# yang-song/score_sde_pytorch

Measured on AMD Instinct MI355X. Metric: pc_sampler_images_per_sec, higher is better.
Workload: dtype f32 via 3-way bf16 split, fp32 accumulate (the 1x1 / NIN / Linear GEMMs and the attention forward as exact-fp32 products on the BF16 matrix pipe, fp32 softmax; 3x3 convolutions and the attention backward on the fp32-MFMA kernels); 1 GPU; configs/ve/cifar10_ncsnpp_continuous PC sampler (reverse_diffusion+langevin), batch 256/GPU, N=1000, 32x32; 1 step = 1 PC iteration = 2 U-Net evaluations; batch_per_gpu=256, sde_steps=1000, state_finite=True, matrix_mode=bf16x6, parallelism=replicas x1 (no collectives)

## Files before the change

### score_sde_pytorch_amd/csrc/conv_mfma.hip

```cpp
#include "ssde_common.h"

typedef float f32x16 __attribute__((ext_vector_type(16)));

namespace {

struct ConvGeom {
  int N, Hin, Win, Hout, Wout, Cout, CoutPad;
  int stride, pad;
  int lTW, lTH;
  int tiles_x, tiles_per_img;
  int m_tiles, n_tiles;
};

struct ConvKParams {
  ssde_src main, aux;
  const float* w_main;
  const float* w_aux;
  ConvGeom g;
  const float* bias;
  const float* chan_add;
  int chan_add_ld;
  const float* resid;
  int resid_post;
  float scale;
  float* dst;
  float* gn_part;
  int ksplit;
  unsigned* sync;
};

constexpr int kThreads = 256;
#ifndef SSDE_CONV_BKC64
#define SSDE_CONV_BKC64 16
#endif

constexpr int kSyncSlots = 1 << 17;
__device__ unsigned g_conv_sync[kSyncSlots * 2];

template <int KS, int BKC, int BM, int BN, int TM, int TN, int MAXI>
__device__ __forceinline__ void conv_phase(const ssde_src& s, const float* __restrict__ wpk,
                                           const ConvGeom& g, int stride, int pad, int Hs, int Ws,
                                           int img0, int ty, int tx, int n0, int wm0, int wn0,
                                           f32x16 (&acc)[TM][TN], float* smem, int ks, int ksplit) {
  constexpr int T = KS * KS;
  constexpr int F4 = BKC / 4;
  constexpr int LDA = BKC + 4;
  constexpr int NB8 = BKC / 8;
  const int tid = threadIdx.x;
  const int lane = tid & 63;
  const int li = lane & 31, lh = lane >> 5;
  const int TW = 1 << g.lTW, TH = 1 << g.lTH;
// ... 258 lines not shown
#pragma unroll
      for (int it = 0; it < ITERS; ++it)
#pragma unroll
        for (int k = 0; k < 4; ++k)
          o[it][k] = dp[it] ? __hip_atomic_load(dp[it] + k, __ATOMIC_RELAXED, __HIP_MEMORY_SCOPE_AGENT) : 0.f;
#pragma unroll
      for (int it = 0; it < ITERS; ++it)
#pragma unroll
        for (int k = 0; k < 4; ++k) tp[it][k] += o[it][k];
    }
    if (first) {
      asm volatile("" ::: "memory");
      __builtin_amdgcn_s_waitcnt(0);
      __syncthreads();
      if (threadIdx.x == 0) atomicAdd(sy + 1, 1u);
      return;
    }
    __syncthreads();
    if (threadIdx.x == 0) { sy[0] = 0u; sy[1] = 0u; }
  }
  SsdeEpi e{p.bias, p.chan_add, p.chan_add_ld, p.resid, p.resid_post, p.scale, p.dst, g.Cout, p.gn_part};
  const int gn_entry = p.gn_part ? img0 * g.tiles_per_img + trem : -1;
  const int rpi_log2 = IMGS > 1 ? g.lTW + g.lTH : 30;
  ssde_store_tile<BM, BN, kThreads>(smem, LDT, n0, e, pixfn, gn_entry, rpi_log2, g.N * g.tiles_per_img);
}

struct TileCfg { int bm, bn; };
const TileCfg kTiles[5] = {{0, 0}, {256, 64}, {128, 64}, {64, 64}, {256, 32}};

struct ConvPlan {
  ConvKParams kp;
  int tile;
  int lds_bytes;
  int grid;
  bool has3, has1;
  int bkc;
  int gn_slices;
};

int src_check(const ssde_src& s, const char* what) {
  SSDE_REQUIRE(s.p0 != nullptr && s.c0 > 0, "conv: %s source missing", what);
  SSDE_REQUIRE(s.c0 % 4 == 0 && s.c1 % 4 == 0, "conv: %s channels must be multiples of 4 (got %d,%d)", what, s.c0, s.c1);
  SSDE_REQUIRE(s.c1 == 0 || s.p1 != nullptr, "conv: %s second tensor missing", what);
  SSDE_REQUIRE(s.c1 == 0 || s.c0 % 32 == 0, "conv: %s concat boundary must be a multiple of 32", what);
  if (s.pro_mode == SSDE_PRO_GN || s.pro_mode == SSDE_PRO_GN_SILU) {
    SSDE_REQUIRE(s.gn_groups > 0 && (s.c0 + s.c1) % s.gn_groups == 0 && ((s.c0 + s.c1) / s.gn_groups) % 4 == 0,
                 "conv: %s GroupNorm needs channels-per-group %% 4 == 0", what);
    SSDE_REQUIRE(s.gn_mean && s.gn_rstd && s.gn_gamma && s.gn_beta, "conv: %s GroupNorm pointers missing", what);
  }
  return SSDE_OK;
}

int pow2_floor(int v) { int p = 1; while (p * 2 <= v) p *= 2; return p; }

int halo_px(int bm, int w_out, int h_out, int stride, int ks, int* lTW, int* lTH) {
// ... 55 lines not shown
  } else {
    halo_px(kTiles[tile].bm, a->w_out, a->h_out, 1, 1, &lTW, &lTH);
  }
  const int bm = kTiles[tile].bm, bn = kTiles[tile].bn;
  const int tw = 1 << lTW, th = 1 << lTH, imgs = bm / (tw * th);

  ConvKParams& kp = pl->kp;
  kp.main = a->main; kp.aux = a->aux; kp.w_main = a->w_main; kp.w_aux = a->w_aux;
  ConvGeom& g = kp.g;
  g.N = a->n; g.Hin = a->h_in; g.Win = a->w_in; g.Hout = a->h_out; g.Wout = a->w_out;
  g.Cout = a->c_out; g.CoutPad = ssde_cdiv(a->c_out, 64) * 64;
  g.stride = pl->has3 ? a->stride : 1; g.pad = pl->has3 ? a->pad : 0;
  g.lTW = lTW; g.lTH = lTH;
  g.tiles_x = ssde_cdiv(a->w_out, tw);
  g.tiles_per_img = g.tiles_x * ssde_cdiv(a->h_out, th);
  g.m_tiles = ssde_cdiv(a->n, imgs) * g.tiles_per_img;
  g.n_tiles = ssde_cdiv(a->c_out, bn);
  kp.bias = a->bias; kp.chan_add = a->chan_add; kp.chan_add_ld = a->chan_add_ld;
  kp.resid = a->resid; kp.resid_post = a->resid_post; kp.scale = a->out_scale; kp.dst = a->dst;
  kp.gn_part = a->gn_part;
  const bool gn_ok = a->c_out % 4 == 0 && (imgs == 1 || (g.tiles_per_img == 1 && tw * th >= kThreads / (bn / 4)));
  pl->gn_slices = gn_ok ? g.tiles_per_img * (kThreads / 64) : 0;
  SSDE_REQUIRE(!a->gn_part || pl->gn_slices > 0, "conv: GroupNorm partials need one image per tile and c_out %% 4 == 0");

  int lds = 0;
  if (pl->has3) {
    const int px = imgs * ((th - 1) * g.stride + 3) * ((tw - 1) * g.stride + 3);
    const int lda = pl->bkc + 4;
    lds = (((px * lda + 3) & ~3) + 9 * bn * lda) * 4;
  }
  if (pl->has1) {
    const int l1 = (bm * 36 + bn * 36) * 4;
    if (l1 > lds) lds = l1;
  }
  const int epi_bytes = bm * (bn + 4) * 4 + 16;
  pl->lds_bytes = lds > epi_bytes ? lds : epi_bytes;
  pl->tile = tile;
  const bool split_ok = !(a->flags & SSDE_CONVF_NO_KSPLIT);
  const int wgs = ssde_cdiv(g.m_tiles, 8) * 8 * g.n_tiles;
  const int ctot = pl->has3 ? a->main.c0 + a->main.c1 : 0;
  kp.ksplit = (split_ok && pl->has3 && tile == SSDE_TILE_64x64 && wgs <= 320 && ctot >= 128 && a->c_out % 4 == 0 &&
               a->resid != a->dst && g.m_tiles * g.n_tiles <= kSyncSlots / 4) ? 2 : 1;
  kp.sync = nullptr;
  pl->grid = wgs * kp.ksplit;
  return SSDE_OK;
}

template <int WM, int WN, int TM, int TN, int BKC3 = 8>
int launch_cfg(ConvPlan& pl, hipStream_t st) {
  dim3 grid(pl.grid), block(kThreads);
  if (pl.kp.ksplit == 2) {
    pl.kp.sync = ssde_conv_sync_slots(pl.kp.g.m_tiles * pl.kp.g.n_tiles);
    SSDE_REQUIRE(pl.kp.sync, "conv: no hand-over slots for a split reduction");
  }
#define SSDE_CONV_LAUNCH(H3, H1)                                                                     \
  do {                                                                                               \
    auto kfn = conv_mfma_kernel<WM, WN, TM, TN, H3, H1, BKC3>;                                       \
    static std::atomic<bool> attr_set{false};             \
// ... 83 lines not shown
}

extern "C" int ssde_conv_gn_slices(const ssde_conv_args* a) {
  if (!a || a->c_out % 4 != 0) return 0;
  if (wino_pad_end_ok(a)) return 0;
  ssde_conv_args q = *a;
  q.gn_part = nullptr;
  if (ssde_wino_launcher fn = wino_launcher(q.tile)) {
    int s = 0;
    if (fn(&q, reinterpret_cast<void*>(1), &s)) return 0;
    return s;
  }
  if (q.dst && ssde_conv1x1_wants(&q)) {
    const int hw = q.h_out * q.w_out;
    if (hw % 64 == 0) return (hw / 64) * 4;
    return (hw >= 8 && hw < 64 && 64 % hw == 0) ? 4 : 0;
  }
  if (q.dst && ssde_conv_small_wants(&q)) return 0;
  ConvPlan pl;
  if (make_plan(&q, &pl)) return 0;
  return pl.gn_slices;
}

extern "C" int64_t ssde_conv_ws_floats(const ssde_conv_args* a) {
  if (int rc = wino_pad_end_ok(a)) return rc;
  if (a && a->tile == SSDE_TILE_WINOGRAD4P) return ssde_conv_wino4p_ws_floats(a);
  return 0;
}

extern "C" int ssde_conv_lds_bytes(const ssde_conv_args* a) {
  if (int rc = wino_pad_end_ok(a)) return rc;
  if (ssde_wino_launcher fn = a ? wino_launcher(a->tile) : nullptr) {
    int lds = 0;
    if (int rc = fn(a, nullptr, &lds)) return rc;
    return lds;
  }
  if (a && a->dst && ssde_conv1x1_wants(a)) {
    int lds = 0;
    if (int rc = ssde_conv1x1_launch(a, nullptr, &lds)) return rc;
    return lds;
  }
  if (a && a->dst && ssde_conv_small_wants(a)) {
    int lds = 0;
    if (int rc = ssde_conv_small_launch(a, nullptr, &lds)) return rc;
    return lds;
  }
// ... 5 lines not shown
```

### score_sde_pytorch_amd/csrc/conv_wino4p.hip

```cpp
#include "ssde_common.h"
#include <type_traits>

namespace {

typedef float f32x16 __attribute__((ext_vector_type(16)));

constexpr int kGemmWaves = 4;
constexpr int kBM = 64, kBN = 64;
constexpr int kKC = 4;
constexpr int kOutLdt = kBN + 4;

struct Wino4pGemmParams {
  const float* v;
  const float* u;
  float* m;
  int T, Q, Np, m_tiles, n_tiles, ks, qper;
};

__global__ __launch_bounds__(64 * kGemmWaves) void wino4p_gemm_kernel(const Wino4pGemmParams p) {
  const int lane = threadIdx.x & 63;
  int r = __builtin_amdgcn_readfirstlane((int)blockIdx.x * kGemmWaves + (int)(threadIdx.x >> 6));
  const int nt = r % p.n_tiles; r /= p.n_tiles;
  const int mt = r % p.m_tiles; r /= p.m_tiles;
  const int pos = r % 36, ks = r / 36;
// ... 101 lines not shown
#pragma unroll
  for (int px = 0; px < 6; ++px) {
    const float m0 = mm[px], m1 = mm[6 + px], m2 = mm[12 + px], m3 = mm[18 + px], m4 = mm[24 + px], m5 = mm[30 + px];
    const float s1 = m1 + m2, d1 = m1 - m2, s2 = m3 + m4, d2 = m3 - m4;
    const float tt[4] = {m0 + s1 + s2, d1 + 2.f * d2, s1 + 4.f * s2, d1 + 8.f * d2 + m5};
#pragma unroll
    for (int dy = 0; dy < 4; ++dy)
#pragma unroll
      for (int dx = 0; dx < 4; ++dx)
        if (kA[px][dx] != 0.f) y[dy][dx] += kA[px][dx] * tt[dy];
  }
#pragma unroll
  for (int dy = 0; dy < 4; ++dy)
#pragma unroll
    for (int dx = 0; dx < 4; ++dx) park[(dy * 4 + dx) * kOutLdt + lane] = y[dy][dx];
  SSDE_LDS_BARRIER();
  const int img = t / p.per_img, tr = t - img * p.per_img;
  const int ty = tr / p.tiles_w, tx = tr - ty * p.tiles_w;
  auto pixfn = [&](int row, size_t& pix, int& im) {
    im = img;
    pix = ((size_t)img * p.H + ty * 4 + (row >> 2)) * p.W + tx * 4 + (row & 3);
    return true;
  };
  ssde_store_tile<16, kBN, 64, 4, 0>(park, kOutLdt, n0, p.e, pixfn, p.e.gn_part ? t : -1);
}

struct W4pShape {
  int T, Q, Np, ks;
  int64_t v_floats;
  int64_t slab_floats;
};

bool w4p_legal_split(int Q, int ks) { return Q % (2 * kKC * ks) == 0; }

int w4p_splits(int waves1, int Q, unsigned flags) {
  if (flags & SSDE_CONVF_NO_KSPLIT) return 1;
  int ks = 1;
  if (flags & (SSDE_CONVF_KSPLIT2 | SSDE_CONVF_KSPLIT4)) {
    ks = (flags & SSDE_CONVF_KSPLIT4) ? 4 : 2;
  } else {
    const int simds = 4 * ssde_num_cus();
    ks = 4;
    while (ks > 1 && (waves1 * ks > simds || Q / ks < 8 * kKC)) ks /= 2;
  }
  while (ks > 1 && !w4p_legal_split(Q, ks)) ks /= 2;
  return ks;
}
// ... 17 lines not shown
  s->Np = ssde_cdiv(a->c_out, kBN) * kBN;
  s->ks = w4p_splits(36 * ssde_cdiv(s->T, kBM) * (s->Np / kBN), s->Q, a->flags);
  s->v_floats = (int64_t)36 * s->T * ctot;
  s->slab_floats = (int64_t)36 * s->T * s->Np;
  return SSDE_OK;
}

}

int64_t ssde_conv_wino4p_ws_floats(const ssde_conv_args* a) {
  W4pShape s;
  if (int rc = w4p_shape(a, &s)) return rc;
  return s.v_floats + s.ks * s.slab_floats;
}

int ssde_conv_wino4p_launch(const ssde_conv_args* a, void* stream, int* lds_out) {
  W4pShape s;
  if (int rc = w4p_shape(a, &s)) return rc;
  const int per_img = (a->h_out / 4) * (a->w_out / 4);
  if (lds_out && stream == reinterpret_cast<void*>(1)) {
    *lds_out = per_img;
    return SSDE_OK;
  }
  const int lds = 16 * kOutLdt * 4;
  if (lds_out) { *lds_out = lds; return SSDE_OK; }
  while (s.ks > 1 && a->wino_ws_floats < s.v_floats + s.ks * s.slab_floats) s.ks /= 2;
  SSDE_REQUIRE(a->wino_ws && a->wino_ws_floats >= s.v_floats + s.ks * s.slab_floats,
               "conv(winograd 4x4, position-batched): workspace (ssde_conv_args.wino_ws) missing or smaller than %lld floats",
               (long long)(s.v_floats + s.slab_floats));
  float* v = a->wino_ws;
  float* m = a->wino_ws + s.v_floats;
  ssde_conv_args x = *a;
  x.wino_v = v;
  if (int rc = ssde_wino4_xform_vq_launch(&x, stream)) return rc;
  hipStream_t st = static_cast<hipStream_t>(stream);
  const Wino4pGemmParams g{v, a->w_main, m, s.T, s.Q, s.Np, ssde_cdiv(s.T, kBM), s.Np / kBN, s.ks, s.Q / s.ks};
  const int waves = 36 * g.m_tiles * g.n_tiles * s.ks;
  hipLaunchKernelGGL(wino4p_gemm_kernel, dim3(ssde_cdiv(waves, kGemmWaves)), dim3(64 * kGemmWaves), 0, st, g);
  SSDE_LAUNCH_CHECK();
  Wino4pOutParams o;
  o.m = m; o.T = s.T; o.Np = s.Np; o.ks = s.ks;
  o.H = a->h_out; o.W = a->w_out; o.tiles_w = a->w_out / 4; o.per_img = per_img;
  o.e = SsdeEpi{a->bias, a->chan_add, a->chan_add_ld, a->resid, a->resid_post, a->out_scale, a->dst, a->c_out, a->gn_part};
  hipLaunchKernelGGL(wino4p_out_kernel, dim3(s.T, s.Np / kBN), dim3(64), lds, st, o);
  SSDE_LAUNCH_CHECK();
  return SSDE_OK;
}
```

### score_sde_pytorch_amd/csrc/conv_wino4r.hip

```cpp
#include "ssde_common.h"
#include <atomic>
#include <type_traits>

typedef float f32x16 __attribute__((ext_vector_type(16)));

#ifdef SSDE_W4R_TRACE
__device__ unsigned long long* g_w4r_trace;
extern "C" int ssde_debug_w4r_trace(void* buf) {
  return hipMemcpyToSymbol(HIP_SYMBOL(g_w4r_trace), &buf, sizeof(buf)) == hipSuccess ? 0 : -5;
}
#define SSDE_RT(slot)                                                                                     \
  do {                                                                                                    \
    if (tr_on) g_w4r_trace[tr_base + (slot)] = __builtin_amdgcn_s_memtime();                              \
  } while (0)
#else
#define SSDE_RT(slot) do { } while (0)
#endif

namespace {

constexpr int kNP = 9;
constexpr int kNV = 5;
constexpr int kPos = 36, kTiles = 32;
constexpr int kURegion = kNP * 32 * 4;
constexpr int kUFloats = 8 * kURegion;
constexpr int kWaves = 8, kThreads = 64 * kWaves, kBN = 64;
constexpr int kLdm = kBN + 2, kLdt = kBN + 4;
constexpr int kLds = kPos * 16 * kLdm * 4;
static_assert(256 * kLdt <= kPos * 16 * kLdm, "parked tile");

struct Wino4rParams {
  const float* v;
  const float* wpk;
  int N, H, W, Cout, Ctot;
  int lTWt, lTHt;
  int tiles_x, tiles_per_img, m_tiles, n_tiles;
  const float* bias; const float* chan_add; int chan_add_ld;
  const float* resid; int resid_post;
  float scale;
  float* dst;
  float* gn_part;
  int T, tiles_h, tiles_w;
  int ksplit;
  unsigned* sync;
  int ticket_off;
};

template <int kKs>
__global__ __launch_bounds__(kThreads, 2) void conv_wino4r_kernel(const Wino4rParams p) {
  constexpr bool kSplit = kKs > 1;
  SSDE_LDS(smem);
  const int tid = threadIdx.x, lane = tid & 63;
  const int wave = __builtin_amdgcn_readfirstlane(tid >> 6);
  const int li = lane & 31, lh = lane >> 5;
  auto pos_of = [&](int i) { return i < 4 ? 4 * wave + i : 32 + (wave >> 1); };
  const int TWt = 1 << p.lTWt, THt = 1 << p.lTHt;
  const int IMGS = kTiles >> (p.lTWt + p.lTHt);
  const size_t v_stage = (size_t)p.T * 16;
  const size_t u_stage = (size_t)p.n_tiles * kUFloats * 4;
  const uint32_t u_off = (uint32_t)lane * 16u, u_off8 = 2048u + (uint32_t)lane * 8u;
  ssde_f32x2 va[2][kNV], u2[2];
  ssde_f32x4 u4[2][4];
  uint32_t v_off[kNV];
  const char* vs = nullptr;
  const char* us = nullptr;
#define SSDE_W4R_ROUND_AT(S, VN, UN)                                                               \
  do {                                                                                             \
    SSDE_GLOAD8_I_SAFE(va[S][0], v_off[0], VN, 0); SSDE_GLOAD16_I_SAFE(u4[S][0], u_off, UN, -2048);          \
// ... 80 lines not shown
    SSDE_W4R_POS(S, 3, 1024);
    SSDE_WAIT_VMCNT_FOR(kMode == 0 ? 18 : kMode == 1 ? 10 : 0, va[S][4], u2[S]);
    SSDE_W4R_MFMA(S, 4, 8, u2[S].x, u2[S].y);
    __builtin_amdgcn_sched_barrier(0);
    if (kMode == 0) { SSDE_W4R_LOADV(S, 4); SSDE_GLOAD8_I(u2[S], u_off8, un, 0); }
    __builtin_amdgcn_sched_barrier(0);
  };
  {
    using S0 = std::integral_constant<int, 0>; using S1 = std::integral_constant<int, 1>;
    using Steady = std::integral_constant<int, 0>; using Penult = std::integral_constant<int, 1>; using Last = std::integral_constant<int, 2>;
    int st = 0;
    for (; st + 3 < nst; st += 2) { stage(S0{}, Steady{}, st); stage(S1{}, Steady{}, st + 1); }
    stage(S0{}, Penult{}, st);
    stage(S1{}, Last{}, st + 1);
  }
#undef SSDE_W4R_POS
#undef SSDE_W4R_MFMA
#undef SSDE_W4R_LOADV
  SSDE_RT(3);

  SsdeEpi e{p.bias, p.chan_add, p.chan_add_ld, p.resid, p.resid_post, p.scale, p.dst, p.Cout, p.gn_part};
  const int gn_base = !p.gn_part ? -1 : (IMGS == 1 ? (img0 * p.tiles_per_img + trem) * 2 : img0);
  const int rpi_log2 = IMGS > 2 ? 8 - (4 - p.lTWt - p.lTHt) : 30;
  const int li_e = tid & 31, lh_e = (tid >> 5) & 1;
  const int e_tl = tid / (kBN / 2), e_cp = tid % (kBN / 2);
  float* park = smem;
#pragma unroll
  for (int rnd = 0; rnd < 2; ++rnd) {
    auto pixfn = [&](int row, size_t& pix, int& img) {
      const int tile = rnd * 16 + (row >> 4), dy = (row >> 2) & 3, dx = row & 3;
      const int il = tile >> (p.lTWt + p.lTHt);
      const int tr = (tile >> p.lTWt) & (THt - 1), tc = tile & (TWt - 1);
      img = img0 + il;
      const int oy = (ty * THt + tr) * 4 + dy, ox = (tx * TWt + tc) * 4 + dx;
      if (img >= p.N || oy >= p.H || ox >= p.W) return false;
      pix = ((size_t)img * p.H + oy) * p.W + ox;
      return true;
    };
#pragma unroll
    for (int j = 0; j < kNP; ++j)
#pragma unroll
      for (int r8 = 0; r8 < 8; ++r8) {
        const int r = rnd * 8 + r8;
        const int tl = (r & 3) + 4 * lh_e + 8 * ((r >> 2) & 1);
        const int pos = pos_of(j >> 1), half = j < 8 ? (j & 1) : (wave & 1);
        smem[(pos * 16 + tl) * kLdm + half * 32 + li_e] = acc[j][r];
// ... 128 lines not shown
  SSDE_REQUIRE((s.c0 + s.c1) % 8 == 0, "conv(winograd 4x4, register-fed): input channels must be a multiple of 8 (the stage loop runs in pairs)");
  Wino4rParams p;
  p.v = a->wino_v; p.wpk = a->w_main;
  p.N = a->n; p.H = a->h_out; p.W = a->w_out; p.Cout = a->c_out; p.Ctot = s.c0 + s.c1;
  const int twt = pow2_floor((a->w_out / 4) < 8 ? (a->w_out / 4) : 8);
  int tht = kTiles / twt; if (tht > a->h_out / 4) tht = a->h_out / 4;
  tht = pow2_floor(tht);
  const int imgs = kTiles / (twt * tht);
  p.lTWt = ssde_ilog2(twt); p.lTHt = ssde_ilog2(tht);
  p.tiles_x = ssde_cdiv(a->w_out, 4 * twt);
  p.tiles_per_img = p.tiles_x * ssde_cdiv(a->h_out, 4 * tht);
  p.m_tiles = ssde_cdiv(a->n, imgs) * p.tiles_per_img;
  p.n_tiles = ssde_cdiv(a->c_out, kBN);
  p.bias = a->bias; p.chan_add = a->chan_add; p.chan_add_ld = a->chan_add_ld;
  p.resid = a->resid; p.resid_post = a->resid_post; p.scale = a->out_scale; p.dst = a->dst;
  p.gn_part = a->gn_part;
  p.tiles_h = a->h_out / 4; p.tiles_w = a->w_out / 4; p.T = a->n * p.tiles_h * p.tiles_w;
  const bool gn_ok = a->c_out % 4 == 0 && (imgs == 1 || (p.tiles_per_img == 1 && imgs <= 8));
  SSDE_REQUIRE(!a->gn_part || gn_ok, "conv(winograd 4x4, register-fed): GroupNorm partials not available for this tiling");
  if (lds_out && stream == reinterpret_cast<void*>(1)) {
    *lds_out = gn_ok ? (imgs == 1 ? 2 * p.tiles_per_img : 1) * (kThreads / 64) : 0;
    return SSDE_OK;
  }
  p.ticket_off = kLds / 4;
  const int lds = kLds + 16;
  SSDE_REQUIRE(lds <= 160 * 1024, "conv(winograd 4x4, register-fed): %d bytes of LDS", lds);
  if (lds_out) { *lds_out = lds; return SSDE_OK; }
  SSDE_REQUIRE(a->wino_v, "conv(winograd 4x4, register-fed): the transformed-input buffer (ssde_conv_args.wino_v) is missing");
  SSDE_REQUIRE(36ull * (unsigned long long)p.T * (unsigned)p.Ctot * 4ull < (1ull << 32),
               "conv(winograd 4x4, register-fed): a transformed input of 4 GB or more is not addressable by this kernel");
  const int wgs = ssde_cdiv(p.m_tiles, 8) * 8 * p.n_tiles;
  p.ksplit = a->resid != a->dst ? ssde_conv_wino4r_splits(wgs, p.Ctot, a->c_out, a->flags) : 1;
  p.sync = p.ksplit > 1 ? ssde_conv_sync_slots(p.m_tiles * p.n_tiles) : nullptr;
  if (!p.sync) p.ksplit = 1;
  const dim3 grid(wgs * p.ksplit);
  auto go = [&](auto kfn, std::atomic<bool>& attr_set) {
    if (!attr_set) {
      if (hipFuncSetAttribute(reinterpret_cast<const void*>(kfn), hipFuncAttributeMaxDynamicSharedMemorySize, 160 * 1024) != hipSuccess)
        return false;
      attr_set = true;
    }
    hipLaunchKernelGGL(kfn, grid, dim3(kThreads), lds, static_cast<hipStream_t>(stream), p);
    return true;
  };
  static std::atomic<bool> set[3];
  const bool ok = p.ksplit == 4 ? go(conv_wino4r_kernel<4>, set[2]) : p.ksplit == 2 ? go(conv_wino4r_kernel<2>, set[1])
// ... 6 lines not shown
```

### score_sde_pytorch_amd/csrc/runtime.hip

```cpp
#include "ssde_common.h"
#include <string.h>
#include <vector>

static thread_local char g_err[512] = "";

void ssde_set_error(const char* fmt, ...) {
  va_list ap;
  va_start(ap, fmt);
  vsnprintf(g_err, sizeof(g_err), fmt, ap);
  va_end(ap);
}

extern "C" const char* ssde_last_error(void) { return g_err; }

int ssde_num_cus() {
  if (const char* e = getenv("SSDE_NUM_CUS")) { const int v = atoi(e); if (v > 0) return v; }
  constexpr int kMaxDev = 64;
  static std::atomic<int> cus[kMaxDev];
  int dev = 0;
  if (hipGetDevice(&dev) != hipSuccess || dev < 0 || dev >= kMaxDev) dev = 0;
  int c = cus[dev].load(std::memory_order_relaxed);
  if (c <= 0) {
    int v = 0;
    if (hipDeviceGetAttribute(&v, hipDeviceAttributeMultiprocessorCount, dev) != hipSuccess || v <= 0) v = 256;
// ... 50 lines not shown
    case SSDE_OP_COLSUM: return ssde_colsum(&op.u.colsum, stream);
    case SSDE_OP_GN_BWD_REDUCE: return ssde_gn_bwd_reduce(&op.u.gn_bwd, stream);
    case SSDE_OP_PROLOGUE_BWD: return ssde_prologue_bwd(&op.u.pro_bwd, stream);
    case SSDE_OP_ATTN_BWD: return ssde_attention_bwd(&op.u.attn_bwd, stream);
    case SSDE_OP_PERTURB: return ssde_perturb(&op.u.perturb, stream);
    case SSDE_OP_DSM_LOSS: return ssde_dsm_loss(&op.u.dsm_loss, stream);
    case SSDE_OP_SUMSQ_FLAT: return ssde_sumsq_flat(&op.u.sumsq_flat, stream);
    case SSDE_OP_ADAM: return ssde_adam_clip_ema(&op.u.adam, stream);
    case SSDE_OP_MEMSET: return ssde_memset(&op.u.memset, stream);
    case SSDE_OP_AXPY: return ssde_axpy(&op.u.axpy, stream);
    case SSDE_OP_PACK: return ssde_pack_weights(&op.u.pack, stream);
    case SSDE_OP_GN_FINALIZE: return ssde_gn_finalize(&op.u.gn_fin, stream);
    case SSDE_OP_PF_DRIFT: return ssde_pf_drift(&op.u.pf_drift, stream);
    case SSDE_OP_HUTCH_DIV: return ssde_hutch_div(&op.u.hutch_div, stream);
    case SSDE_OP_COLSUM_FINISH: return ssde_colsum_finish(&op.u.colsum_fin, stream);
    case SSDE_OP_GN_BWD_FINISH: return ssde_gn_bwd_finish(&op.u.gn_bwd_fin, stream);
    case SSDE_OP_GN_APPLY: return ssde_gn_apply(&op.u.gn_apply, stream);
    case SSDE_OP_GN_APPLY_BWD: return ssde_gn_apply_bwd(&op.u.gn_apply_bwd, stream);
  }
  ssde_set_error("program: unknown op kind %d", op.kind);
  return SSDE_EINVAL;
}

extern "C" int ssde_program_run(const ssde_op* ops, int32_t n_ops, void* stream) {
  SSDE_REQUIRE(ops && n_ops >= 0, "program: null ops");
  for (int i = 0; i < n_ops; ++i) {
    if (int rc = run_one(ops[i], stream)) {
      char tmp[400];
      strncpy(tmp, g_err, sizeof(tmp) - 1); tmp[sizeof(tmp) - 1] = 0;
      ssde_set_error("op %d (kind %d): %s", i, ops[i].kind, tmp);
      return rc;
    }
  }
  return SSDE_OK;
}

extern "C" int ssde_program_run_timed(const ssde_op* ops, int32_t n_ops, void* stream, float* ms) {
  SSDE_REQUIRE(ops && n_ops >= 0 && ms, "program: null args");
  hipStream_t st = static_cast<hipStream_t>(stream);
  std::vector<hipEvent_t> ev(n_ops + 1);
  for (auto& e : ev) SSDE_HIP_CHECK(hipEventCreate(&e));
  int rc = SSDE_OK;
  SSDE_HIP_CHECK(hipEventRecord(ev[0], st));
  for (int i = 0; i < n_ops && rc == SSDE_OK; ++i) {
    rc = run_one(ops[i], stream);
    if (rc == SSDE_OK && hipEventRecord(ev[i + 1], st) != hipSuccess) { ssde_set_error("hipEventRecord failed"); rc = SSDE_EHIP; }
  }
  if (rc == SSDE_OK) {
    if (hipStreamSynchronize(st) != hipSuccess) { ssde_set_error("hipStreamSynchronize failed"); rc = SSDE_EHIP; }
    for (int i = 0; i < n_ops && rc == SSDE_OK; ++i)
      if (hipEventElapsedTime(&ms[i], ev[i], ev[i + 1]) != hipSuccess) { ssde_set_error("hipEventElapsedTime failed"); rc = SSDE_EHIP; }
  }
  for (auto& e : ev) hipEventDestroy(e);
  return rc;
}

struct SsdeGraph { hipGraph_t graph; hipGraphExec_t exec; };

extern "C" int ssde_graph_capture(const ssde_op* ops, int32_t n_ops, void* stream, void** graph_out) {
  SSDE_REQUIRE(ops && graph_out, "graph: null args");
  hipStream_t st = static_cast<hipStream_t>(stream);
  SSDE_REQUIRE(st != nullptr, "graph: capture needs a non-default stream");
  SSDE_HIP_CHECK(hipStreamBeginCapture(st, hipStreamCaptureModeThreadLocal));
  int rc = ssde_program_run(ops, n_ops, stream);
  hipGraph_t graph = nullptr;
  hipError_t e = hipStreamEndCapture(st, &graph);
  if (rc != SSDE_OK) { if (graph) hipGraphDestroy(graph); return rc; }
  if (e != hipSuccess) { ssde_set_error("hipStreamEndCapture failed: %s", hipGetErrorString(e)); return SSDE_EHIP; }
  hipGraphExec_t exec = nullptr;
// ... 23 lines not shown
```

### score_sde_pytorch_amd/csrc/ssde_common.h

```cpp
#pragma once
#include <hip/hip_runtime.h>
#include <stdint.h>
#include <stdio.h>
#include <stdarg.h>
#include <stdlib.h>
#include <atomic>
#include "../../include/ssde.h"

#define SSDE_OK 0
#define SSDE_EINVAL (-22)
#define SSDE_EHIP (-5)

void ssde_set_error(const char* fmt, ...);
int ssde_conv_wino_launch(const ssde_conv_args* a, void* stream, int* lds_out);
int ssde_conv_wino4_launch(const ssde_conv_args* a, void* stream, int* lds_out);
bool ssde_wino4_xform_merges_gn(const ssde_conv_args* a);
int ssde_wino4_xform_vq_launch(const ssde_conv_args* a, void* stream);
int ssde_conv_wino4r_launch(const ssde_conv_args* a, void* stream, int* lds_out);
int ssde_conv_wino4p_launch(const ssde_conv_args* a, void* stream, int* lds_out);
int64_t ssde_conv_wino4p_ws_floats(const ssde_conv_args* a);
bool ssde_conv1x1_wants(const ssde_conv_args* a);
int ssde_conv1x1_launch(const ssde_conv_args* a, void* stream, int* lds_out);
unsigned* ssde_conv_sync_slots(int need);
int ssde_conv_wino4_splits(int wgs, int ctot, int c_out, unsigned flags);
int ssde_conv_wino4r_splits(int wgs, int ctot, int c_out, unsigned flags);
bool ssde_conv_small_wants(const ssde_conv_args* a);
int ssde_conv_small_launch(const ssde_conv_args* a, void* stream, int* lds_out);
bool ssde_wgrad_wino_wants(const ssde_wgrad_args* a);
int64_t ssde_wgrad_wino_scratch_floats(const ssde_wgrad_args* a);
int ssde_wgrad_wino_launch(const ssde_wgrad_args* a, void* stream);
bool ssde_wgrad_wino4_wants(const ssde_wgrad_args* a);
int64_t ssde_wgrad_wino4_scratch_floats(const ssde_wgrad_args* a);
int ssde_wgrad_wino4_launch(const ssde_wgrad_args* a, void* stream);

#define SSDE_REQUIRE(cond, ...)            \
  do {                                     \
    if (!(cond)) {                         \
      ssde_set_error(__VA_ARGS__);         \
      return SSDE_EINVAL;                  \
    }                                      \
  } while (0)

#define SSDE_HIP_CHECK(expr)                                                        \
  do {                                                                              \
    hipError_t _e = (expr);                                                         \
// ... 129 lines not shown
__device__ __forceinline__ float ssde_keep(uint32_t elem, const SsdePro& p) {
  return ssde_hash32(elem * 0x9E3779B1u + p.key) >= p.thresh ? p.dscale : 0.f;
}
__device__ __forceinline__ float4 ssde_pro_apply(float4 v, float mu, float rs, const float4& gam, const float4& bet,
                                                 uint32_t elem0, const SsdePro& p) {
  if (p.gn) {
    v.x = (v.x - mu) * rs * gam.x + bet.x;
    v.y = (v.y - mu) * rs * gam.y + bet.y;
    v.z = (v.z - mu) * rs * gam.z + bet.z;
    v.w = (v.w - mu) * rs * gam.w + bet.w;
  }
  if (p.silu) { v.x = ssde_silu(v.x); v.y = ssde_silu(v.y); v.z = ssde_silu(v.z); v.w = ssde_silu(v.w); }
  if (__builtin_expect(p.drop, 0)) {
    v.x *= ssde_keep(elem0, p); v.y *= ssde_keep(elem0 + 1u, p);
    v.z *= ssde_keep(elem0 + 2u, p); v.w *= ssde_keep(elem0 + 3u, p);
  }
  return v;
}

struct SsdeEpi {
  const float* bias; const float* chan_add; int chan_add_ld;
  const float* resid; int resid_post; float scale; float* dst; int Cout;
  float* gn_part = nullptr;
};

__device__ __forceinline__ void ssde_stat_merge(float& n, float& m, float& M2, float nb, float mb, float M2b) {
#pragma clang fp contract(off)
  const float nt = n + nb;
  const float d = mb - m;
  const float f = nt > 0.f ? nb * __builtin_amdgcn_rcpf(nt) : 0.f;
  m += d * f;
  M2 += M2b + d * d * n * f;
  n = nt;
}
struct SsdeGnTeam {
  const float* part0; const float* part1;
  int Q0, Q1, s0, s1, q0, qm, cpq, e0, etot, n;
  float v[4][3];
  __device__ __forceinline__ const float* entry(int k) const {
    if (k < e0) {
      const int nq = qm - q0, s = k / nq, q = q0 + (k - s * nq);
      return part0 + (((size_t)n * s0 + s) * Q0 + q) * 3;
    }
    const int kk = k - e0, nq = q0 + cpq - qm, s = kk / nq, q = qm - Q0 + (kk - s * nq);
    return part1 + (((size_t)n * s1 + s) * Q1 + q) * 3;
  }
};
// ... 26 lines not shown
  for (int i = 0; i < 4; ++i)
    if (l16 + 16 * i < t.etot) ssde_stat_merge(cnt, m, M2, t.v[i][2], t.v[i][0], t.v[i][1]);
  for (int k = l16 + 64; k < t.etot; k += 16) {
    const float* e = t.entry(k);
    ssde_stat_merge(cnt, m, M2, e[2], e[0], e[1]);
  }
#pragma unroll
  for (int o = 1; o < 16; o <<= 1) {
    const float nb = __shfl_xor(cnt, o, 64), mb = __shfl_xor(m, o, 64), Mb = __shfl_xor(M2, o, 64);
    if (l16 & o) { float tn = nb, tm = mb, tM = Mb; ssde_stat_merge(tn, tm, tM, cnt, m, M2); cnt = tn; m = tm; M2 = tM; }
    else ssde_stat_merge(cnt, m, M2, nb, mb, Mb);
  }
}
__device__ __forceinline__ float ssde_gn_rstd(float cnt, float M2, float eps) {
#pragma clang fp contract(off)
  const float var = cnt > 0.f ? M2 / cnt : 0.f;
  return 1.0f / sqrtf(var + eps);
}
__device__ __forceinline__ void ssde_gn_merge16(const float* part0, const float* part1, int c0, int c1, int s0, int s1, int groups,
                                                int n, int g, int l16, float& cnt, float& m, float& M2) {
  SsdeGnTeam t;
  ssde_gn_merge16_load(t, part0, part1, c0, c1, s0, s1, groups, n, g, l16);
  ssde_gn_merge16_finish(t, l16, cnt, m, M2);
}

template <int ROWS, int NCOLS, int NT, int BATCH = 4, int SWZ = 0, class PixFn>
__device__ __forceinline__ void ssde_store_tile(float* tile, int ld, int n0, const SsdeEpi& e, PixFn pixfn, int gn_entry = -1,
                                                int rpi_log2 = 30, int gn_entry_max = 0x7fffffff) {
  const int tidx = threadIdx.x;
  constexpr int C4N = NCOLS / 4, TOTAL = ROWS * C4N, ITERS = TOTAL / NT, RSTEP = NT / C4N;
  static_assert(TOTAL % NT == 0 && NT % C4N == 0 && 64 % C4N == 0, "a thread owns one channel quad of ITERS rows");
  const int c = (tidx % C4N) * 4, row0 = tidx / C4N;
  const int j = n0 + c;
  const bool stats = e.gn_part != nullptr && gn_entry >= 0;
  float st_p = 0.f, st_s1 = 0.f, st_s2 = 0.f, st_n = 0.f;
  const int rpi_mask = (rpi_log2 < 30 ? (1 << rpi_log2) : ROWS) - 1;
  auto flush = [&](int it) {
    float n = st_n, m = 0.f, M2 = 0.f;
    if (n > 0.f) { const float rn = __builtin_amdgcn_rcpf(n); m = st_p + st_s1 * rn; M2 = st_s2 - st_s1 * st_s1 * rn; M2 = M2 < 0.f ? 0.f : M2; }
    for (int o = C4N; o < 64; o <<= 1) {
      const float nb = __shfl_xor(n, o, 64), mb = __shfl_xor(m, o, 64), Mb = __shfl_xor(M2, o, 64);
      if (tidx & o) { float tn = nb, tm = mb, tM = Mb; ssde_stat_merge(tn, tm, tM, n, m, M2); n = tn; m = tm; M2 = tM; }
      else ssde_stat_merge(n, m, M2, nb, mb, Mb);
    }
    const int lane = tidx & 63, wave = tidx >> 6;
    const int entry = gn_entry + ((it * RSTEP) >> (rpi_log2 < 30 ? rpi_log2 : 30));
    if (lane < C4N && n0 + 4 * lane < e.Cout && entry < gn_entry_max) {
      float* o = e.gn_part + (((size_t)entry * (NT / 64) + wave) * (e.Cout >> 2) + (n0 >> 2) + lane) * 3;
      o[0] = m; o[1] = M2; o[2] = n;
    }
    st_p = st_s1 = st_s2 = st_n = 0.f;
  };
  if ((e.Cout & 3) == 0) {
    const bool col_ok = j < e.Cout;
    float4 bias4 = make_float4(0.f, 0.f, 0.f, 0.f);
    if (e.bias && col_ok) bias4 = *reinterpret_cast<const float4*>(e.bias + j);
    constexpr int B = ITERS >= BATCH ? BATCH : ITERS;
    static_assert(ITERS % B == 0, "row batches");
#pragma unroll
    for (int it0 = 0; it0 < ITERS; it0 += B) {
      float4 t[B], r[B], a[B];
      size_t pix[B];
      bool ok[B];
#pragma unroll
      for (int b = 0; b < B; ++b) {
        const int row = row0 + (it0 + b) * RSTEP;
        int img = 0;
        pix[b] = 0;
        ok[b] = col_ok && pixfn(row, pix[b], img);
        t[b] = *reinterpret_cast<const float4*>(tile + row * ld + (SWZ ? (c ^ (((row >> 4) & 1) << 4)) : c));
        r[b] = make_float4(0.f, 0.f, 0.f, 0.f);
        a[b] = make_float4(0.f, 0.f, 0.f, 0.f);
        if (ok[b] && e.resid) r[b] = *reinterpret_cast<const float4*>(e.resid + pix[b] * e.Cout + j);
// ... 29 lines not shown
#else
#pragma unroll
      for (int b = 0; b < B; ++b) {
        if (ok[b]) {
          float v[4] = {t[b].x + bias4.x + a[b].x, t[b].y + bias4.y + a[b].y, t[b].z + bias4.z + a[b].z, t[b].w + bias4.w + a[b].w};
          const float4 rr = r[b];
          if (!e.resid_post) { v[0] += rr.x; v[1] += rr.y; v[2] += rr.z; v[3] += rr.w; }
#pragma unroll
          for (int k = 0; k < 4; ++k) v[k] *= e.scale;
          if (e.resid_post) { v[0] += rr.x; v[1] += rr.y; v[2] += rr.z; v[3] += rr.w; }
          *reinterpret_cast<float4*>(e.dst + pix[b] * e.Cout + j) = make_float4(v[0], v[1], v[2], v[3]);
          if (stats) {
            if (st_n == 0.f) st_p = v[0];
            const float d0 = v[0] - st_p, d1 = v[1] - st_p, d2 = v[2] - st_p, d3 = v[3] - st_p;
            st_s1 += (d0 + d1) + (d2 + d3);
            st_s2 += (d0 * d0 + d1 * d1) + (d2 * d2 + d3 * d3);
            st_n += 4.f;
          }
        }
        if (stats && (((it0 + b + 1) * RSTEP) & rpi_mask) == 0) flush(it0 + b);
      }
#endif
    }
  } else {
    for (int it = 0; it < ITERS; ++it) {
      const int row = row0 + it * RSTEP;
      size_t pix; int img;
      if (j >= e.Cout || !pixfn(row, pix, img)) continue;
      const float4 t = *reinterpret_cast<const float4*>(tile + row * ld + (SWZ ? (c ^ (((row >> 4) & 1) << 4)) : c));
      const float v[4] = {t.x, t.y, t.z, t.w};
      for (int k = 0; k < 4 && j + k < e.Cout; ++k) {
        float x = v[k];
        if (e.bias) x += e.bias[j + k];
        if (e.chan_add) x += e.chan_add[(size_t)img * e.chan_add_ld + j + k];
        const float r = e.resid ? e.resid[pix * e.Cout + j + k] : 0.f;
        if (e.resid && !e.resid_post) x += r;
        x *= e.scale;
        if (e.resid && e.resid_post) x += r;
        e.dst[pix * e.Cout + j + k] = x;
      }
    }
  }
}


typedef __bf16 ssde_bf16x8 __attribute__((ext_vector_type(8)));
// ... 45 lines not shown
```

Measured before the change: 5.631 images/s.

## Fuse GroupNorm statistics finalize into the producing convolution epilogue

When a conv op that emits GroupNorm partials is immediately followed by a GN_FINALIZE op, the runtime now runs them as one launch. The conv epilogue parks the per-wave partials in LDS, merges them per group and writes the final mean/rstd directly. This removes a separate finalize kernel launch and its re-read of the partials. It only applies when a tile covers whole groups of a whole image and no buffers alias. It costs extra LDS and an extra barrier in the epilogue, and it can be switched off with an environment variable.

```diff
diff --git a/score_sde_pytorch_amd/csrc/conv_mfma.hip b/score_sde_pytorch_amd/csrc/conv_mfma.hip
--- a/score_sde_pytorch_amd/csrc/conv_mfma.hip
+++ b/score_sde_pytorch_amd/csrc/conv_mfma.hip
@@ -27,6 +27,7 @@
   float* gn_part;
   int ksplit;
   unsigned* sync;
+  SsdeGnFinish fin;
 };
 
 constexpr int kThreads = 256;
@@ -331,6 +332,7 @@
   SsdeEpi e{p.bias, p.chan_add, p.chan_add_ld, p.resid, p.resid_post, p.scale, p.dst, g.Cout, p.gn_part};
   const int gn_entry = p.gn_part ? img0 * g.tiles_per_img + trem : -1;
   const int rpi_log2 = IMGS > 1 ? g.lTW + g.lTH : 30;
+  if (p.fin.mean) ssde_epi_set_finish(e, p.fin, smem + BM * LDT + 4);
   ssde_store_tile<BM, BN, kThreads>(smem, LDT, n0, e, pixfn, gn_entry, rpi_log2, g.N * g.tiles_per_img);
 }
 
@@ -340,6 +342,7 @@
 struct ConvPlan {
   ConvKParams kp;
   int tile;
+  bool fin_ok;
   int lds_bytes;
   int grid;
   bool has3, has1;
@@ -441,6 +444,10 @@
   const bool gn_ok = a->c_out % 4 == 0 && (imgs == 1 || (g.tiles_per_img == 1 && tw * th >= kThreads / (bn / 4)));
   pl->gn_slices = gn_ok ? g.tiles_per_img * (kThreads / 64) : 0;
   SSDE_REQUIRE(!a->gn_part || pl->gn_slices > 0, "conv: GroupNorm partials need one image per tile and c_out %% 4 == 0");
+  const ssde_gn_finalize_args* fin = ssde_gn_finish_request();
+  pl->fin_ok = gn_ok && g.tiles_per_img == 1 && ssde_gn_finish_fits(a, fin, true, kThreads / 64, bn);
+  SSDE_REQUIRE(!fin || !a->gn_part || pl->fin_ok, "conv: this tiling cannot finish the GroupNorm statistics of its output");
+  kp.fin = (fin && a->gn_part) ? ssde_gn_finish_of(fin) : SsdeGnFinish{};
 
   int lds = 0;
   if (pl->has3) {
@@ -452,7 +459,7 @@
     const int l1 = (bm * 36 + bn * 36) * 4;
     if (l1 > lds) lds = l1;
   }
-  const int epi_bytes = bm * (bn + 4) * 4 + 16;
+  const int epi_bytes = bm * (bn + 4) * 4 + 16 + (kp.fin.mean ? imgs * (kThreads / 64) * (bn / 4) * 3 * 4 : 0);
   pl->lds_bytes = lds > epi_bytes ? lds : epi_bytes;
   pl->tile = tile;
   const bool split_ok = !(a->flags & SSDE_CONVF_NO_KSPLIT);
@@ -582,6 +589,22 @@
   return pl.gn_slices;
 }
 
+bool ssde_conv_finishes_gn(const ssde_conv_args* a, const ssde_gn_finalize_args* f) {
+  if (!a || !f || !a->gn_part || a->c_out % 4 != 0 || wino_pad_end_ok(a)) return false;
+  const ssde_gn_finalize_args* prev = ssde_gn_finish_request_swap(f);
+  int yes = 0;
+  if (a->tile == SSDE_TILE_WINOGRAD4R || a->tile == SSDE_TILE_WINOGRAD4P) {
+    if (wino_launcher(a->tile)(a, reinterpret_cast<void*>(2), &yes)) yes = 0;
+  } else if (wino_launcher(a->tile) || (a->dst && (ssde_conv1x1_wants(a) || ssde_conv_small_wants(a)))) {
+    yes = 0;
+  } else {
+    ConvPlan pl;
+    yes = make_plan(a, &pl) == SSDE_OK && pl.fin_ok;
+  }
+  ssde_gn_finish_request_swap(prev);
+  return yes != 0;
+}
+
 extern "C" int64_t ssde_conv_ws_floats(const ssde_conv_args* a) {
   if (int rc = wino_pad_end_ok(a)) return rc;
   if (a && a->tile == SSDE_TILE_WINOGRAD4P) return ssde_conv_wino4p_ws_floats(a);
diff --git a/score_sde_pytorch_amd/csrc/conv_wino4p.hip b/score_sde_pytorch_amd/csrc/conv_wino4p.hip
--- a/score_sde_pytorch_amd/csrc/conv_wino4p.hip
+++ b/score_sde_pytorch_amd/csrc/conv_wino4p.hip
@@ -147,7 +147,9 @@
     pix = ((size_t)img * p.H + ty * 4 + (row >> 2)) * p.W + tx * 4 + (row & 3);
     return true;
   };
-  ssde_store_tile<16, kBN, 64, 4, 0>(park, kOutLdt, n0, p.e, pixfn, p.e.gn_part ? t : -1);
+  SsdeEpi e = p.e;
+  if (e.fin_mean) e.fin_lds = park + 16 * kOutLdt;
+  ssde_store_tile<16, kBN, 64, 4, 0>(park, kOutLdt, n0, e, pixfn, e.gn_part ? t : -1);
 }
 
 struct W4pShape {
@@ -211,7 +213,12 @@
     *lds_out = per_img;
     return SSDE_OK;
   }
-  const int lds = 16 * kOutLdt * 4;
+  const ssde_gn_finalize_args* fin = ssde_gn_finish_request();
+  const bool fin_ok = per_img == 1 && ssde_gn_finish_fits(a, fin, true, 1, kBN);
+  if (lds_out && stream == reinterpret_cast<void*>(2)) { *lds_out = fin_ok ? 1 : 0; return SSDE_OK; }
+  SSDE_REQUIRE(!fin || !a->gn_part || fin_ok, "conv(winograd 4x4, position-batched): this tiling cannot finish the GroupNorm statistics of its output");
+  const bool finishing = fin && a->gn_part;
+  const int lds = 16 * kOutLdt * 4 + (finishing ? (kBN / 4) * 3 * 4 : 0);
   if (lds_out) { *lds_out = lds; return SSDE_OK; }
   while (s.ks > 1 && a->wino_ws_floats < s.v_floats + s.ks * s.slab_floats) s.ks /= 2;
   SSDE_REQUIRE(a->wino_ws && a->wino_ws_floats >= s.v_floats + s.ks * s.slab_floats,
@@ -231,6 +238,7 @@
   o.m = m; o.T = s.T; o.Np = s.Np; o.ks = s.ks;
   o.H = a->h_out; o.W = a->w_out; o.tiles_w = a->w_out / 4; o.per_img = per_img;
   o.e = SsdeEpi{a->bias, a->chan_add, a->chan_add_ld, a->resid, a->resid_post, a->out_scale, a->dst, a->c_out, a->gn_part};
+  if (finishing) ssde_epi_set_finish(o.e, ssde_gn_finish_of(fin), nullptr);
   hipLaunchKernelGGL(wino4p_out_kernel, dim3(s.T, s.Np / kBN), dim3(64), lds, st, o);
   SSDE_LAUNCH_CHECK();
   return SSDE_OK;
diff --git a/score_sde_pytorch_amd/csrc/conv_wino4r.hip b/score_sde_pytorch_amd/csrc/conv_wino4r.hip
--- a/score_sde_pytorch_amd/csrc/conv_wino4r.hip
+++ b/score_sde_pytorch_amd/csrc/conv_wino4r.hip
@@ -28,6 +28,8 @@
 constexpr int kLdm = kBN + 2, kLdt = kBN + 4;
 constexpr int kLds = kPos * 16 * kLdm * 4;
 static_assert(256 * kLdt <= kPos * 16 * kLdm, "parked tile");
+constexpr int kFinOff = 256 * kLdt;
+static_assert(kFinOff + 4 * kWaves * (kBN / 4) * 3 <= kPos * 16 * kLdm, "parked partials");
 
 struct Wino4rParams {
   const float* v;
@@ -44,6 +46,7 @@
   int ksplit;
   unsigned* sync;
   int ticket_off;
+  SsdeGnFinish fin;
 };
 
 template <int kKs>
@@ -170,6 +173,7 @@
   SsdeEpi e{p.bias, p.chan_add, p.chan_add_ld, p.resid, p.resid_post, p.scale, p.dst, p.Cout, p.gn_part};
   const int gn_base = !p.gn_part ? -1 : (IMGS == 1 ? (img0 * p.tiles_per_img + trem) * 2 : img0);
   const int rpi_log2 = IMGS > 2 ? 8 - (4 - p.lTWt - p.lTHt) : 30;
+  if (p.fin.mean) ssde_epi_set_finish(e, p.fin, smem + kFinOff);
   const int li_e = tid & 31, lh_e = (tid >> 5) & 1;
   const int e_tl = tid / (kBN / 2), e_cp = tid % (kBN / 2);
   float* park = smem;
@@ -344,6 +348,11 @@
     *lds_out = gn_ok ? (imgs == 1 ? 2 * p.tiles_per_img : 1) * (kThreads / 64) : 0;
     return SSDE_OK;
   }
+  const ssde_gn_finalize_args* fin = ssde_gn_finish_request();
+  const bool fin_ok = gn_ok && imgs >= 2 && ssde_gn_finish_fits(a, fin, true, kThreads / 64, kBN);
+  if (lds_out && stream == reinterpret_cast<void*>(2)) { *lds_out = fin_ok ? 1 : 0; return SSDE_OK; }
+  SSDE_REQUIRE(!fin || !a->gn_part || fin_ok, "conv(winograd 4x4, register-fed): this tiling cannot finish the GroupNorm statistics of its output");
+  p.fin = (fin && a->gn_part) ? ssde_gn_finish_of(fin) : SsdeGnFinish{};
   p.ticket_off = kLds / 4;
   const int lds = kLds + 16;
   SSDE_REQUIRE(lds <= 160 * 1024, "conv(winograd 4x4, register-fed): %d bytes of LDS", lds);
diff --git a/score_sde_pytorch_amd/csrc/runtime.hip b/score_sde_pytorch_amd/csrc/runtime.hip
--- a/score_sde_pytorch_amd/csrc/runtime.hip
+++ b/score_sde_pytorch_amd/csrc/runtime.hip
@@ -96,10 +96,104 @@
   return SSDE_EINVAL;
 }
 
+static thread_local const ssde_gn_finalize_args* g_fin_request = nullptr;
+const ssde_gn_finalize_args* ssde_gn_finish_request() { return g_fin_request; }
+
+const ssde_gn_finalize_args* ssde_gn_finish_request_swap(const ssde_gn_finalize_args* f) {
+  const ssde_gn_finalize_args* prev = g_fin_request;
+  g_fin_request = f;
+  return prev;
+}
+
+int ssde_conv2d_finishing(const ssde_conv_args* a, const ssde_gn_finalize_args* f, void* stream) {
+  const ssde_gn_finalize_args* prev = ssde_gn_finish_request_swap(f);
+  const int rc = ssde_conv2d(a, stream);
+  ssde_gn_finish_request_swap(prev);
+  return rc;
+}
+
+static std::atomic<int> g_fin_switch{-1};
+static std::atomic<long long> g_fin_count{0};
+static bool fin_enabled() {
+  int v = g_fin_switch.load(std::memory_order_relaxed);
+  if (v < 0) {
+    const char* e = getenv("SSDE_GN_FINISH_IN_PRODUCER");
+    v = (e && e[0] == '0' && e[1] == 0) ? 0 : 1;
+    g_fin_switch.store(v, std::memory_order_relaxed);
+  }
+  return v != 0;
+}
+extern "C" int ssde_debug_gn_finish_switch(int on) {
+  if (on == 0 || on == 1) g_fin_switch.store(on, std::memory_order_relaxed);
+  return fin_enabled() ? 1 : 0;
+}
+extern "C" long long ssde_debug_gn_finish_count(void) { return g_fin_count.load(std::memory_order_relaxed); }
+
+static bool fin_overlaps(const float* w, size_t wn, const void* p, size_t floats) {
+  if (!p || !floats) return false;
+  const char* a0 = reinterpret_cast<const char*>(w);
+  const char* b0 = reinterpret_cast<const char*>(p);
+  return a0 < b0 + floats * 4 && b0 < a0 + wn * 4;
+}
+static bool fin_src_overlaps(const float* w, size_t wn, const ssde_src& s, size_t px) {
+  const size_t c = (size_t)(s.c0 + s.c1);
+  return fin_overlaps(w, wn, s.p0, px * s.c0) || fin_overlaps(w, wn, s.p1, px * s.c1) || fin_overlaps(w, wn, s.gn_gamma, c) ||
+         fin_overlaps(w, wn, s.gn_beta, c) || fin_overlaps(w, wn, s.drop_seed, 1);
+}
+static bool fin_aliases(const ssde_conv_args& c, const ssde_gn_finalize_args& f) {
+  const size_t wn = (size_t)f.n * f.groups, n = (size_t)c.n;
+  const size_t px_in = n * c.h_in * c.w_in, px_out = n * c.h_out * c.w_out;
+  const float* const outs[2] = {f.mean, f.rstd};
+  if (fin_overlaps(f.mean, wn, f.rstd, wn)) return true;
+  for (const float* w : outs) {
+    for (const ssde_src* s : {&c.main, &c.aux}) {
+      if (!s->p0) continue;
+      if (s == &c.main && (c.tile == SSDE_TILE_WINOGRAD4R || c.tile == SSDE_TILE_WINOGRAD4P)) continue;
+      if (fin_src_overlaps(w, wn, *s, s == &c.main ? px_in : px_out)) return true;
+      const size_t st = n * (size_t)(s->gn_groups > 0 ? s->gn_groups : 0);
+      if (fin_overlaps(w, wn, s->gn_mean, st) || fin_overlaps(w, wn, s->gn_rstd, st)) return true;
+    }
+    const size_t in_c = (size_t)(c.main.c0 + c.main.c1), tiles = px_in / 16;
+    if (fin_overlaps(w, wn, c.w_main, 1) || fin_overlaps(w, wn, c.w_aux, 1) || fin_overlaps(w, wn, c.bias, c.c_out) ||
+        fin_overlaps(w, wn, c.chan_add, n * (size_t)c.chan_add_ld) || fin_overlaps(w, wn, c.resid, px_out * c.c_out) ||
+        fin_overlaps(w, wn, c.dst, px_out * c.c_out) || fin_overlaps(w, wn, c.gn_part, n * (size_t)f.slices0 * (c.c_out / 4) * 3) ||
+        fin_overlaps(w, wn, c.wino_v, 36 * tiles * in_c) || fin_overlaps(w, wn, c.wino_ws, c.wino_ws_floats > 0 ? (size_t)c.wino_ws_floats : 0) ||
+        fin_overlaps(w, wn, c.gn_in_part0, n * (size_t)(c.gn_in_slices0 > 0 ? c.gn_in_slices0 : 0) * (c.main.c0 / 4) * 3) ||
+        fin_overlaps(w, wn, c.gn_in_part1, n * (size_t)(c.gn_in_slices1 > 0 ? c.gn_in_slices1 : 0) * (c.main.c1 / 4) * 3))
+      return true;
+  }
+  return false;
+}
+
+static bool fin_pair(const ssde_op* ops, int i, int n_ops) {
+  if (i + 1 >= n_ops || ops[i].kind != SSDE_OP_CONV || ops[i + 1].kind != SSDE_OP_GN_FINALIZE || !fin_enabled()) return false;
+  const ssde_conv_args& c = ops[i].u.conv;
+  const ssde_gn_finalize_args& f = ops[i + 1].u.gn_fin;
+  if (!c.gn_part || f.part0 != c.gn_part || f.part1 != nullptr || f.c1 != 0 || !f.mean || !f.rstd) return false;
+  if (f.c0 != c.c_out || f.n != c.n || f.slices0 != ssde_conv_gn_slices(&c)) return false;
+  return ssde_conv_finishes_gn(&c, &f) && !fin_aliases(c, f);
+}
+extern "C" int ssde_debug_gn_finish_pairs(const ssde_op* ops, int32_t n_ops) {
+  int pairs = 0;
+  for (int i = 0; ops && i + 1 < n_ops; ++i)
+    if (fin_pair(ops, i, n_ops)) { ++pairs; ++i; }
+  return pairs;
+}
+
+static int run_at(const ssde_op* ops, int i, int n_ops, void* stream, int* took) {
+  *took = 1;
+  if (fin_pair(ops, i, n_ops)) {
+    *took = 2;
+    g_fin_count.fetch_add(1, std::memory_order_relaxed);
+    return ssde_conv2d_finishing(&ops[i].u.conv, &ops[i + 1].u.gn_fin, stream);
+  }
+  return run_one(ops[i], stream);
+}
+
 extern "C" int ssde_program_run(const ssde_op* ops, int32_t n_ops, void* stream) {
   SSDE_REQUIRE(ops && n_ops >= 0, "program: null ops");
-  for (int i = 0; i < n_ops; ++i) {
-    if (int rc = run_one(ops[i], stream)) {
+  for (int i = 0, took = 1; i < n_ops; i += took) {
+    if (int rc = run_at(ops, i, n_ops, stream, &took)) {
       char tmp[400];
       strncpy(tmp, g_err, sizeof(tmp) - 1); tmp[sizeof(tmp) - 1] = 0;
       ssde_set_error("op %d (kind %d): %s", i, ops[i].kind, tmp);
@@ -116,9 +210,10 @@
   for (auto& e : ev) SSDE_HIP_CHECK(hipEventCreate(&e));
   int rc = SSDE_OK;
   SSDE_HIP_CHECK(hipEventRecord(ev[0], st));
-  for (int i = 0; i < n_ops && rc == SSDE_OK; ++i) {
-    rc = run_one(ops[i], stream);
-    if (rc == SSDE_OK && hipEventRecord(ev[i + 1], st) != hipSuccess) { ssde_set_error("hipEventRecord failed"); rc = SSDE_EHIP; }
+  for (int i = 0, took = 1; i < n_ops && rc == SSDE_OK; i += took) {
+    rc = run_at(ops, i, n_ops, stream, &took);
+    for (int k = 1; k <= took && rc == SSDE_OK; ++k)
+      if (hipEventRecord(ev[i + k], st) != hipSuccess) { ssde_set_error("hipEventRecord failed"); rc = SSDE_EHIP; }
   }
   if (rc == SSDE_OK) {
     if (hipStreamSynchronize(st) != hipSuccess) { ssde_set_error("hipStreamSynchronize failed"); rc = SSDE_EHIP; }
diff --git a/score_sde_pytorch_amd/csrc/ssde_common.h b/score_sde_pytorch_amd/csrc/ssde_common.h
--- a/score_sde_pytorch_amd/csrc/ssde_common.h
+++ b/score_sde_pytorch_amd/csrc/ssde_common.h
@@ -21,6 +21,10 @@
 int64_t ssde_conv_wino4p_ws_floats(const ssde_conv_args* a);
 bool ssde_conv1x1_wants(const ssde_conv_args* a);
 int ssde_conv1x1_launch(const ssde_conv_args* a, void* stream, int* lds_out);
+const ssde_gn_finalize_args* ssde_gn_finish_request();
+const ssde_gn_finalize_args* ssde_gn_finish_request_swap(const ssde_gn_finalize_args* f);
+bool ssde_conv_finishes_gn(const ssde_conv_args* a, const ssde_gn_finalize_args* f);
+int ssde_conv2d_finishing(const ssde_conv_args* a, const ssde_gn_finalize_args* f, void* stream);
 unsigned* ssde_conv_sync_slots(int need);
 int ssde_conv_wino4_splits(int wgs, int ctot, int c_out, unsigned flags);
 int ssde_conv_wino4r_splits(int wgs, int ctot, int c_out, unsigned flags);
@@ -196,7 +200,13 @@
   const float* bias; const float* chan_add; int chan_add_ld;
   const float* resid; int resid_post; float scale; float* dst; int Cout;
   float* gn_part = nullptr;
+  float* fin_mean = nullptr; float* fin_rstd = nullptr; int fin_groups = 0; float fin_eps = 0.f;
+  float* fin_lds = nullptr;
 };
+struct SsdeGnFinish { float* mean = nullptr; float* rstd = nullptr; int groups = 0; float eps = 0.f; };
+__host__ __device__ __forceinline__ void ssde_epi_set_finish(SsdeEpi& e, const SsdeGnFinish& f, float* lds) {
+  e.fin_mean = f.mean; e.fin_rstd = f.rstd; e.fin_groups = f.groups; e.fin_eps = f.eps; e.fin_lds = lds;
+}
 
 __device__ __forceinline__ void ssde_stat_merge(float& n, float& m, float& M2, float nb, float mb, float M2b) {
 #pragma clang fp contract(off)
@@ -269,6 +279,49 @@
   SsdeGnTeam t;
   ssde_gn_merge16_load(t, part0, part1, c0, c1, s0, s1, groups, n, g, l16);
   ssde_gn_merge16_finish(t, l16, cnt, m, M2);
+}
+
+static inline bool ssde_gn_finish_fits(const ssde_conv_args* a, const ssde_gn_finalize_args* f, bool whole, int nw, int bn) {
+  if (!a || !f || !whole || f->groups <= 0 || a->c_out % 4 != 0 || a->c_out % f->groups != 0) return false;
+  const int w = a->c_out / f->groups;
+  return w % 4 == 0 && bn % w == 0 && nw * (w / 4) <= 64;
+}
+static inline SsdeGnFinish ssde_gn_finish_of(const ssde_gn_finalize_args* f) {
+  SsdeGnFinish r;
+  if (f) { r.mean = f->mean; r.rstd = f->rstd; r.groups = f->groups; r.eps = f->eps; }
+  return r;
+}
+template <int ROWS, int NCOLS, int NT>
+__device__ __forceinline__ void ssde_gn_finish_tile(const SsdeEpi& e, int n0, int gn_entry, int rpi_log2, int gn_entry_max) {
+  constexpr int C4N = NCOLS / 4, NW = NT / 64, TEAMS = NT / 16;
+  SSDE_LDS_BARRIER();
+  const int imgs = rpi_log2 < 30 ? ROWS >> rpi_log2 : 1;
+  const int cpq = (e.Cout / e.fin_groups) >> 2;
+  const int gpt = C4N / cpq;
+  const int pairs = imgs * gpt;
+  const int team = threadIdx.x >> 4, l16 = threadIdx.x & 15;
+  SsdeGnTeam t;
+  t.part0 = t.part1 = nullptr;
+  t.Q0 = t.Q1 = t.s0 = t.s1 = t.q0 = t.qm = t.e0 = t.n = 0;
+  t.cpq = cpq; t.etot = NW * cpq;
+  for (int p0 = 0; p0 < pairs; p0 += TEAMS) {
+    const int pi = p0 + team < pairs ? p0 + team : pairs - 1;
+    const int il = pi / gpt, gl = pi - il * gpt;
+#pragma unroll
+    for (int i = 0; i < 4; ++i) {
+      const int k = l16 + 16 * i < t.etot ? l16 + 16 * i : 0;
+      const int s = k / cpq, q = gl * cpq + (k - s * cpq);
+      const float* v = e.fin_lds + ((il * NW + s) * C4N + q) * 3;
+      t.v[i][0] = v[0]; t.v[i][1] = v[1]; t.v[i][2] = v[2];
+    }
+    float cnt, m, M2;
+    ssde_gn_merge16_finish(t, l16, cnt, m, M2);
+    const int n = gn_entry + il, g = (n0 >> 2) / cpq + gl;
+    if (l16 == 0 && p0 + team < pairs && n < gn_entry_max && g < e.fin_groups) {
+      e.fin_mean[(size_t)n * e.fin_groups + g] = m;
+      e.fin_rstd[(size_t)n * e.fin_groups + g] = ssde_gn_rstd(cnt, M2, e.fin_eps);
+    }
+  }
 }
 
 template <int ROWS, int NCOLS, int NT, int BATCH = 4, int SWZ = 0, class PixFn>
@@ -296,6 +349,11 @@
       float* o = e.gn_part + (((size_t)entry * (NT / 64) + wave) * (e.Cout >> 2) + (n0 >> 2) + lane) * 3;
       o[0] = m; o[1] = M2; o[2] = n;
     }
+    if (e.fin_mean && lane < C4N) {
+      const int il = rpi_log2 < 30 ? (it * RSTEP) >> rpi_log2 : 0;
+      float* s = e.fin_lds + ((il * (NT / 64) + wave) * C4N + lane) * 3;
+      s[0] = m; s[1] = M2; s[2] = n;
+    }
     st_p = st_s1 = st_s2 = st_n = 0.f;
   };
   if ((e.Cout & 3) == 0) {
@@ -371,6 +429,7 @@
       }
 #endif
     }
+    if (stats && e.fin_mean) ssde_gn_finish_tile<ROWS, NCOLS, NT>(e, n0, gn_entry, rpi_log2, gn_entry_max);
   } else {
     for (int it = 0; it < ITERS; ++it) {
       const int row = row0 + it * RSTEP;
```

Result: no change. 5.616 images/s (-0.3%).
